# ru1ven/KeypointFusion

Hardware: AMD Instinct MI355X
Metric: RGB-D img/sec fwd (B=64, 256x256) (higher is better)
Workload: dtype f32; 1 GPU; KPFusion-convnext-tiny, depth+RGB UNet backbones forward, B=64/GPU 256x256 f32 (BASELINE configs[1]); batch_per_gpu=64, global_batch=64, input=256x256, parallelism=dp1 (batch shards, no collective)

## Files before the change

include/kpf.h:

```cpp
#ifndef KPF_H
#define KPF_H

#ifdef __cplusplus
extern "C" {
#endif

#define KPF_OK 0
#define KPF_EINVAL (-1)
#define KPF_ELAUNCH (-2)

#define KPF_DT_F32 0
#define KPF_DT_BF16 1
#define KPF_DT_F16 2
#define KPF_DT_F32_MMA_BF16 8
#define KPF_DT_F32_MMA_F16 9

#define KPF_ACT_RELU 1u
#define KPF_ACT_GELU 2u
#define KPF_RES_ADD 4u
#define KPF_RES_GAMMA 8u
#define KPF_RELU_AFTER_RES 16u
#define KPF_ACT_LEAKY 64u
#define KPF_IN_SPLIT 128u
#define KPF_W_SPLIT 512u
// ... 320 lines not shown
int kpf_geom_gate_uvd_forward(const float* pix_xyz, const float* joint_uvd, const float* par16, float* gam, int B, int J, int P, float half_size, float flip,
                              void* stream);
int kpf_geom_gate_uvd_backward(const float* pix_xyz, const float* joint_uvd, const float* par16, const float* dgam, float* djoint_uvd, int B, int J, int P,
                               float half_size, float flip, void* stream);

int kpf_prep_crop_u16(const unsigned char* rgb, const unsigned short* depth, const double* bbox, const double* cam, const double* cube, int B, int Hs, int Ws,
                      int x0, int y0, int H, int W, int S, float* img, float* img_rgb, float* center, float* M, float* cube_out, float* cam_para, double* com,
                      int* bounds, double* M64, void* stream);

int kpf_prep_pcl_sample(const float* img, const float* center, const double* M64, const double* cube, const double* cam, const long long* seed, int B, int S,
                        int n, float* pcl, int* pcl_index, int* pcl_count, float* cand_pts, void* stream);

int kpf_prep_uncrop_f32(const float* joints, const float* center, const float* M, const float* cube, const float* cam, int B, int J, float* crop_px,
                        float* frame_px, void* stream);

int kpf_prep_set_stamps(void* stamps64 );

int kpf_eval_errors_f32(const float* const* stages, int S, const float* gt, const float* cube, const int* score_index, int B, int J, int Jsel, float* err,
                        void* stream);

int kpf_eval_accumulate(const float* err, const unsigned char* valid, const double* thresholds, int S, int B, int Jsel, int T, long long* n_samples,
                        long long* n_batches, double* sum_err, double* sum_pa, double* sum_batch_mean, double* sum_batch_pa_mean, long long* pck,
                        long long* pck_pa, void* stream);

int kpf_prep_crop_u16_indexed(const unsigned char* rgb, const unsigned short* depth, const int* frame_index, int F, const double* bbox, const double* cam,
                              const double* cube, int B, int Hs, int Ws, int x0, int y0, int H, int W, int S, float* img, float* img_rgb, float* center, float* M,
                              float* cube_out, float* cam_para, double* com, int* bounds, double* M64, void* stream);

int kpf_track_step_f32(const float* joints, const float* center, const float* M, const float* cube, const float* cam_para, const int* pcl_count, int B, int J,
                       int frame_w, int frame_h, float expansion, long long seed_stride, double* bbox, long long* seed, int* lost, float* crop_px,
                       float* frame_px, float* cam_mm, double* bbox_used, int* status, void* stream);

int kpf_conv_num_tile_cfgs(void);

const char* kpf_last_error(void);
#define KPF_ABI_VERSION 21
int kpf_abi_version(void);

#ifdef __cplusplus
}
#endif
#endif
```

keypointfusion_amd/csrc/kpf_conv.hip:

```cpp
#include "kpf_common.h"
#include <stdlib.h>
#include <type_traits>

namespace {

struct ConvArgs {
  const float* in;
  const float* w;
  const float* bias;
  const float* ps;
  const float* pt;
  const float* gamma;
  const float* res;
  float* out;
  int M, N, K, Kp;
  int IH, IW, Cin, in_ld, in_coff;
  int OH, OW, ohow, KH, KW, sh, sw, ph, pw;
  int out_ld, out_coff, res_ld, res_coff;
  const float* zero;
  float w_unscale;
  unsigned flags;
  int tilesN, nblk;
  int vec;
  int dbg;
// ... 697 lines not shown
          blk[0] = h;
          blk[32] = (_Float16)(yc - (float)h);
        } else
          a.out[(long)m * a.out_ld + a.out_coff + n + e] = y;
      }
    }
  }
}

template <int TM, int TN, int WM, int WN, bool IS1X1, bool HAS_PRO, int EPI, int NS>
__global__ __launch_bounds__(64 * WM * WN) void igemm_f32_kernel(const ConvArgs a) {
  igemm_body<TM, TN, WM, WN, IS1X1, HAS_PRO, EPI, ARITH_F32, NS>(kpf_group_args(a));
}
template <int TM, int TN, int WM, int WN, bool IS1X1, int EPI, int ARITH>
__global__ __launch_bounds__(64 * WM * WN) void igemm_r16_kernel(const ConvArgs a) {
  igemm_body<TM, TN, WM, WN, IS1X1, false, EPI, ARITH, 2>(kpf_group_args(a));
}
template <int TM, int TN, int WM, int WN, bool IS1X1, bool HAS_PRO, int EPI, int ARITH, int NS>
__global__ __launch_bounds__(64 * WM * WN) void igemm_split_kernel(const ConvArgs a) {
  igemm_body<TM, TN, WM, WN, IS1X1, HAS_PRO, EPI, ARITH, NS>(kpf_group_args(a));
}
template <int TM, int TN, int WM, int WN, bool IS1X1, bool HAS_PRO, int EPI, int ARITH>
__global__ __launch_bounds__(64 * WM * WN, 4) void igemm_split_occ_kernel(const ConvArgs a) {
  igemm_body<TM, TN, WM, WN, IS1X1, HAS_PRO, EPI, ARITH, 1>(kpf_group_args(a));
}

template <int TM, int TN, int WM, int WN, bool IS1X1, bool HAS_PRO, int EPI, int ARITH, int NS>
__global__ __launch_bounds__(64 * WM * WN) void igemm_h16_kernel(const ConvArgs a) {
  igemm_body<TM, TN, WM, WN, IS1X1, HAS_PRO, EPI, ARITH, NS>(kpf_group_args(a));
}
template <int TM, int TN, int WM, int WN, bool IS1X1, bool HAS_PRO, int EPI, int ARITH>
__global__ __launch_bounds__(64 * WM * WN, 4) void igemm_h16_occ_kernel(const ConvArgs a) {
  igemm_body<TM, TN, WM, WN, IS1X1, HAS_PRO, EPI, ARITH, 1>(kpf_group_args(a));
}

template <int TM, int TN, int WM, int WN, bool IS1X1, bool HAS_PRO, int EPI, int ARITH, int NS>
int launch_one(const ConvArgs& a, hipStream_t st) {
  constexpr int BM = 16 * TM * WM, BN = 16 * TN * WN, RPP = 8 * WM * WN;
  constexpr bool R16 = ARITH == ARITH_R_BF16 || ARITH == ARITH_R_F16;
  constexpr bool WHOLE = NS > 2 || ARITH == ARITH_F32 || R16;
  constexpr int BMR = WHOLE ? (BM + RPP - 1) / RPP * RPP : BM, BNR = WHOLE ? (BN + RPP - 1) / RPP * RPP : BN;
  constexpr bool H16 = ARITH == ARITH_BF16 || ARITH == ARITH_F16;
  size_t lds = (size_t)(NS * (BMR + BNR) * BK + (HAS_PRO ? 2 * a.Kp * (H16 ? 2 : 1) : 0)) * sizeof(float);
  if (H16 && EPI != EPI_RES && EPI != EPI_GGRAD && TN == 4) {
    const size_t stg = (size_t)WM * WN * TM * 16 * (TN * 16 + 8) * 2;
    if (stg > lds) lds = stg;
  }
  void (*kern)(const ConvArgs);
  if constexpr (ARITH == ARITH_F32)
    kern = igemm_f32_kernel<TM, TN, WM, WN, IS1X1, HAS_PRO, EPI, NS>;
  else if constexpr (R16)
    kern = igemm_r16_kernel<TM, TN, WM, WN, IS1X1, EPI, ARITH>;
  else if constexpr (H16 && NS == 1)
    kern = igemm_h16_occ_kernel<TM, TN, WM, WN, IS1X1, HAS_PRO, EPI, ARITH>;
  else if constexpr (H16)
    kern = igemm_h16_kernel<TM, TN, WM, WN, IS1X1, HAS_PRO, EPI, ARITH, NS>;
  else if constexpr (NS == 1)
    kern = igemm_split_occ_kernel<TM, TN, WM, WN, IS1X1, HAS_PRO, EPI, ARITH>;
  else
    kern = igemm_split_kernel<TM, TN, WM, WN, IS1X1, HAS_PRO, EPI, ARITH, NS>;
  static std::atomic<bool> lds_opt_in[KPF_MAX_DEVICES];
  if (!kpf_raise_lds_limit(reinterpret_cast<const void*>(kern), lds_opt_in)) {
    kpf_set_error("kpf_conv2d_f32: cannot raise the dynamic LDS limit");
    return KPF_ELAUNCH;
  }
  if (lds > 160 * 1024) {
// ... 600 lines not shown
    }
  }
  static const bool no_kxk = getenv("KPF_NO_KXK16") != nullptr;
  if (!no_kxk && !pointwise && !pro_scale && a.groups <= 1 && !(fl & (KPF_RES_GELU_GRAD | KPF_ACT_GELU_SAVE | KPF_OUT_NCHW)) && a.M >= 16384) {
    const long tm256 = ((long)a.M + 255) / 256;
    if (a.N % 256 == 0 && tm256 * (a.N / 256) >= 256) best = 26;
    else if (a.N % 128 == 0 && tm256 * (a.N / 128) >= 256) best = 8;
    else if (a.N == 64) best = 2;
  }
  static const int forced = []() { const char* e = getenv("KPF_FORCE_CFG16"); return e ? atoi(e) : -1; }();
  if (forced >= 0 && (forced != 30 || ok8)) best = forced;
  if (d->tile_cfg > 0 && (d->tile_cfg != 31 || ok8)) best = d->tile_cfg - 1;
  if (best == 30) return dtype == KPF_DT_BF16 ? launch_8ph<ARITH_BF16>(a, st) : launch_8ph<ARITH_F16>(a, st);
#ifdef KPF_FAST_BUILD
  return launch_cfg_h16<4, 4, 2, 2, 2>(a, fast1x1, pointwise, dtype, st);
#endif
  switch (best) {
    case 0: return occ ? launch_cfg_h16<4, 4, 2, 2, 1>(a, fast1x1, pointwise, dtype, st) : launch_cfg_h16<4, 4, 2, 2, 2>(a, fast1x1, pointwise, dtype, st);
    case 1: return launch_cfg_h16<4, 3, 2, 2, 2>(a, fast1x1, pointwise, dtype, st);
    case 2: return launch_cfg_h16<2, 4, 4, 1, 2>(a, fast1x1, pointwise, dtype, st);
    case 5: return launch_cfg_h16<2, 4, 2, 2, 2>(a, fast1x1, pointwise, dtype, st);
    case 6: return occ ? launch_cfg_h16<2, 2, 2, 2, 1>(a, fast1x1, pointwise, dtype, st) : launch_cfg_h16<2, 2, 2, 2, 2>(a, fast1x1, pointwise, dtype, st);
    case 8: return launch_cfg_h16<4, 4, 4, 2, 2>(a, fast1x1, pointwise, dtype, st);
    case 20: return launch_cfg_h16<4, 4, 4, 2, 3>(a, fast1x1, pointwise, dtype, st);
    case 21: return launch_cfg_h16<4, 4, 2, 2, 3>(a, fast1x1, pointwise, dtype, st);
    case 22: return launch_cfg_h16<4, 4, 2, 2, 4>(a, fast1x1, pointwise, dtype, st);
    case 26: return launch_cfg_h16<8, 4, 2, 4, 2>(a, fast1x1, pointwise, dtype, st);
    case 41: return launch_cfg_h16<2, 2, 2, 2, 4>(a, fast1x1, pointwise, dtype, st);
    case 44: return launch_cfg_h16<2, 1, 1, 4, 8>(a, fast1x1, pointwise, dtype, st);
    default: return launch_cfg_h16<2, 1, 1, 4, 2>(a, fast1x1, pointwise, dtype, st);
  }
}
#else
extern "C" int kpf_conv2d_f32(const kpf_conv_desc* d, const float* in, const float* w, const float* bias,
                              const float* pro_scale, const float* pro_shift, const float* gamma, const float* res,
                              float* out, void* stream) {
  KPF_REQUIRE(d && in && w && out, "kpf_conv2d_f32: null pointer");
  KPF_REQUIRE(d->B > 0 && d->OH > 0 && d->OW > 0 && d->N > 0 && d->Cin > 0, "kpf_conv2d_f32: empty shape");
  KPF_REQUIRE(d->Cin % 4 == 0 && d->in_ld % 4 == 0 && d->in_coff % 4 == 0,
              "kpf_conv2d_f32: Cin/in_ld/in_coff must be multiples of 4 (got %d/%d/%d)", d->Cin, d->in_ld, d->in_coff);
  KPF_REQUIRE(d->Kp % 32 == 0 && d->Kp >= d->KH * d->KW * d->Cin, "kpf_conv2d_f32: Kp=%d must be a multiple of 32 and >= K=%d",
              d->Kp, d->KH * d->KW * d->Cin);
  KPF_REQUIRE(kpf_aligned16(in) && kpf_aligned16(w) && kpf_aligned16(out), "kpf_conv2d_f32: pointers must be 16-byte aligned");
  const unsigned fl = d->flags;
  if (!(fl & KPF_OUT_NCHW))
    KPF_REQUIRE(d->out_coff >= 0 && d->out_coff + d->N <= d->out_ld, "kpf_conv2d_f32: bad output slice ld=%d coff=%d N=%d",
                d->out_ld, d->out_coff, d->N);
  if (fl & KPF_RES_ADD)
    KPF_REQUIRE(res && kpf_aligned16(res) && d->res_coff >= 0 && d->res_coff + d->N <= d->res_ld, "kpf_conv2d_f32: bad residual");
  if (fl & KPF_RES_GAMMA) KPF_REQUIRE(gamma && (fl & KPF_RES_ADD), "kpf_conv2d_f32: RES_GAMMA needs gamma and RES_ADD");
  KPF_REQUIRE((pro_scale == nullptr) == (pro_shift == nullptr), "kpf_conv2d_f32: prologue needs both scale and shift");
  KPF_REQUIRE(((fl & KPF_ACT_RELU) != 0) + ((fl & KPF_ACT_GELU) != 0) + ((fl & KPF_ACT_LEAKY) != 0) <= 1, "kpf_conv2d_f32: one activation only");
  KPF_REQUIRE(!((fl & KPF_RES_ADD) && (fl & (KPF_ACT_RELU | KPF_ACT_GELU | KPF_ACT_LEAKY))), "kpf_conv2d_f32: activation before a residual add is not supported");
  KPF_REQUIRE(!((fl & KPF_ACT_LEAKY) && pro_scale), "kpf_conv2d_f32: LeakyReLU is not combined with an operand prologue");
  KPF_REQUIRE(!(fl & KPF_RELU_AFTER_RES) || (fl & KPF_RES_ADD), "kpf_conv2d_f32: RELU_AFTER_RES needs RES_ADD");
  KPF_REQUIRE(!(fl & KPF_RES_GELU_GRAD) || ((fl & KPF_RES_ADD) && !(fl & (KPF_RES_GAMMA | KPF_RELU_AFTER_RES | KPF_OUT_NCHW))), "kpf_conv2d_f32: RES_GELU_GRAD goes with RES_ADD alone");
  KPF_REQUIRE(!(fl & KPF_ACT_GELU_SAVE) || ((fl & KPF_ACT_GELU) && !(fl & (KPF_RES_ADD | KPF_OUT_NCHW)) && res && kpf_aligned16(res) && d->res_coff >= 0 && d->res_coff + d->N <= d->res_ld),
              "kpf_conv2d_f32: ACT_GELU_SAVE goes with ACT_GELU and a second output buffer in the res slot (res_ld / res_coff describe it)");
  KPF_REQUIRE((long)d->B * d->OH * d->OW < (1l << 31) && (long)d->B * d->IH * d->IW < (1l << 31), "kpf_conv2d_f32: too many pixels");

  ConvArgs a;
  a.in = in; a.w = w; a.bias = bias; a.ps = pro_scale; a.pt = pro_shift; a.gamma = gamma; a.res = res; a.out = out;
  a.M = d->B * d->OH * d->OW; a.N = d->N; a.K = d->KH * d->KW * d->Cin; a.Kp = d->Kp;
  a.IH = d->IH; a.IW = d->IW; a.Cin = d->Cin; a.in_ld = d->in_ld; a.in_coff = d->in_coff;
  a.OH = d->OH; a.OW = d->OW; a.ohow = d->OH * d->OW; a.KH = d->KH; a.KW = d->KW;
  a.sh = d->sh; a.sw = d->sw; a.ph = d->ph; a.pw = d->pw;
  a.out_ld = d->out_ld; a.out_coff = d->out_coff; a.res_ld = d->res_ld; a.res_coff = d->res_coff;
  {
    static const float* zero_of_dev[64] = {nullptr};
    int dev = 0;
    if (hipGetDevice(&dev) != hipSuccess || dev < 0 || dev >= 64) dev = 0;
    if (!zero_of_dev[dev]) {
      void* p = nullptr;
      if (hipGetSymbolAddress(&p, HIP_SYMBOL(kpf_zero16)) != hipSuccess || !p) {
        kpf_set_error("kpf_conv2d_f32: cannot resolve the zero page");
        return KPF_ELAUNCH;
      }
      zero_of_dev[dev] = static_cast<const float*>(p);
    }
    a.zero = zero_of_dev[dev];
  }
  a.flags = fl; a.tilesN = 0; a.nblk = 0; a.dbg = 0; a.skew = 0; a.st_policy = 0;
  {
    static const int st_mb = []() { const char* e = getenv("KPF_F32_ST_MB"); return e ? atoi(e) : 0; }();
    if (st_mb > 0 && (long)d->B * d->OH * d->OW * d->N * 4 >= (long)st_mb * 1000000) a.st_policy = 2;
  }
  a.w_unscale = (fl & (KPF_IN_SPLIT | KPF_W_SPLIT)) ? d->w_unscale : 1.0f;
  if (fl & (KPF_IN_SPLIT | KPF_W_SPLIT))
    KPF_REQUIRE(d->w_unscale > 0.f && d->Cin % 32 == 0 && d->in_coff % 4 == 0, "kpf_conv2d_f32: split operands need w_unscale > 0 and Cin %% 32 == 0 (Cin=%d)", d->Cin);
  if (fl & KPF_IN_SPLIT) KPF_REQUIRE(d->in_coff % 32 == 0 && d->in_ld % 32 == 0 && !pro_scale, "kpf_conv2d_f32: split activations need in_ld, in_coff multiples of 32 and no operand prologue");
  if (fl & KPF_OUT_SPLIT)
    KPF_REQUIRE(d->N % 32 == 0 && d->out_coff % 32 == 0 && d->out_ld % 32 == 0 && !(fl & KPF_OUT_NCHW),
                "kpf_conv2d_f32: split output needs N, out_ld, out_coff multiples of 32 (N=%d ld=%d coff=%d)", d->N, d->out_ld, d->out_coff);
  a.vec = (d->out_ld % 4 == 0 && d->out_coff % 4 == 0 && (!(fl & KPF_RES_ADD) || (d->res_ld % 4 == 0 && d->res_coff % 4 == 0))) ? 1 : 0;
  a.groups = d->groups > 1 ? d->groups : 1; a.g_in = a.g_out = 0; a.g_w = 0;
  if (a.groups > 1) {
    KPF_REQUIRE(!(fl & (KPF_RES_GAMMA | KPF_OUT_NCHW | KPF_IN_SPLIT | KPF_W_SPLIT | KPF_OUT_SPLIT)) && !pro_scale && d->w_gstride % 4 == 0,
                "kpf_conv2d_f32: a grouped launch takes no layer scale / prologue / NCHW output / split operands, and needs w_gstride %% 4 == 0");
    KPF_REQUIRE(d->in_coff + d->groups * d->Cin <= d->in_ld && d->out_coff + d->groups * d->N <= d->out_ld, "kpf_conv2d_f32: the groups' channel slices exceed the pixel stride");
    KPF_REQUIRE(!(fl & (KPF_RES_ADD | KPF_ACT_GELU_SAVE)) || d->res_coff + d->groups * d->N <= d->res_ld,
                "kpf_conv2d_f32: the groups' residual / saved pre-activation slices exceed the pixel stride");
    a.g_in = d->Cin; a.g_out = d->N; a.g_w = d->w_gstride;
    if ((d->out_coff + d->N) % 4 || ((fl & KPF_RES_ADD) && (d->res_coff + d->N) % 4)) a.vec = 0;
  }
  const bool is1x1 = d->KH == 1 && d->KW == 1 && d->sh == 1 && d->sw == 1 && d->ph == 0 && d->pw == 0 &&
                     d->IH == d->OH && d->IW == d->OW && d->Cin % 32 == 0 && d->Kp == d->Cin;
  hipStream_t st = reinterpret_cast<hipStream_t>(stream);

  int best = 0;
  double bc = 1e30;
  static const int forced = []() { const char* e = getenv("KPF_FORCE_CFG"); return e ? atoi(e) : -1; }();
  for (int i = 0; i < (int)(sizeof(kCfgs) / sizeof(kCfgs[0])); ++i) {
    const double c = cfg_cost(kCfgs[i], a.M, a.N, a.groups);
    if (c < bc) { bc = c; best = i; }
  }
  const bool f32_arith = !(fl & (KPF_IN_SPLIT | KPF_W_SPLIT));
  const bool gelu1x1 = f32_arith && is1x1 && (fl & KPF_ACT_GELU) && !(fl & KPF_ACT_GELU_SAVE) && !pro_scale && d->groups <= 1;
  if (gelu1x1 && a.M >= 1024 && a.N >= 512) {
    auto rounds_cost = [&](int bm, int bn, double pen) { return (double)((((long)(a.M + bm - 1) / bm) * ((a.N + bn - 1) / bn) + 255) / 256) * bm * bn * pen; };
    const double c0 = rounds_cost(128, 128, 1.00), c8 = rounds_cost(256, 128, 0.97);
    best = c0 <= c8 ? 0 : 8;
  }
  if (f32_arith && best < 9 && a.Kp >= 512) {
    const long bb = ((a.M + kCfgs[best].bm - 1) / kCfgs[best].bm) * ((a.N + kCfgs[best].bn - 1) / kCfgs[best].bn) * a.groups;
    if (bb < 256 && (long)((a.M + 31) / 32) * ((a.N + 63) / 64) * a.groups >= 512) best = 7;
  }
  if ((fl & (KPF_IN_SPLIT | KPF_W_SPLIT)) && !(fl & KPF_RES_ADD) && !pro_scale && (best == 0 || best == 8)) best = 13;
  if ((fl & (KPF_IN_SPLIT | KPF_W_SPLIT)) && !pro_scale && a.Kp >= 1024) {
    const long blocks = ((a.M + kCfgs[best < 9 ? best : 0].bm - 1) / kCfgs[best < 9 ? best : 0].bm) *
                        ((a.N + kCfgs[best < 9 ? best : 0].bn - 1) / kCfgs[best < 9 ? best : 0].bn);
    const long blocks64 = ((a.M + 63) / 64) * ((a.N + 63) / 64);
    if (best < 9 && blocks <= 512 && blocks64 >= 512) best = 16;
  }
  if (forced >= 0) best = forced;
  if (d->tile_cfg > 0) {
    KPF_REQUIRE(d->tile_cfg <= KPF_NUM_TILE_CFGS, "kpf_conv2d_f32: tile_cfg %d out of range", d->tile_cfg);
    best = d->tile_cfg - 1;
  }
#ifdef KPF_FAST_BUILD
  return launch_cfg<4, 4, 2, 2>(a, is1x1, st);
#else
  switch (best) {
    case 0: return launch_cfg<4, 4, 2, 2>(a, is1x1, st);
    case 1: return launch_cfg<4, 3, 2, 2>(a, is1x1, st);
    case 2: return launch_cfg<2, 4, 4, 1>(a, is1x1, st);
    case 3: return launch_cfg<4, 3, 4, 1>(a, is1x1, st);
    case 4: return launch_cfg<2, 7, 4, 1>(a, is1x1, st);
    case 5: return launch_cfg<2, 4, 2, 2>(a, is1x1, st);
    case 6: return launch_cfg<2, 2, 2, 2>(a, is1x1, st);
    case 8: return launch_cfg<4, 4, 4, 2>(a, is1x1, st);
    case 9: return launch_cfg<4, 4, 4, 2, 3>(a, is1x1, st);
    case 10: return launch_cfg<4, 4, 2, 2>(a, is1x1, st);
    case 11: return launch_cfg<4, 3, 2, 2>(a, is1x1, st);
    case 12: return launch_cfg<2, 4, 4, 1, 3>(a, is1x1, st);
    case 13: return launch_cfg<4, 4, 2, 2, 1>(a, is1x1, st);
    case 14: return launch_cfg<4, 3, 2, 2, 1>(a, is1x1, st);
    case 15: return launch_cfg<2, 4, 4, 1, 1>(a, is1x1, st);
    case 16: return launch_cfg<2, 2, 2, 2, 1>(a, is1x1, st);
    case 17: return launch_cfg<4, 6, 2, 2>(a, is1x1, st);
    default: return launch_cfg<2, 1, 1, 4>(a, is1x1, st);
  }
#endif
}

extern "C" int kpf_conv_num_tile_cfgs(void) { return KPF_NUM_TILE_CFGS; }
#endif

#ifdef KPF_DBG_TIME
extern "C" int kpf_dbg_read(unsigned long long* host, int n) {
  return hipMemcpyFromSymbol(host, HIP_SYMBOL(kpf_dbg_t), sizeof(unsigned long long) * n) == hipSuccess ? 0 : -1;
// ... 7 lines not shown
```

keypointfusion_amd/lib.py:

```python
import ctypes as C
import os

_HERE = os.path.dirname(os.path.abspath(__file__))
LIB_PATH = os.environ.get("KPF_LIB_PATH") or os.path.join(_HERE, "libkpf_hip.so")

KPF_ACT_RELU = 1
KPF_ACT_GELU = 2
KPF_RES_ADD = 4
KPF_RES_GAMMA = 8
KPF_RELU_AFTER_RES = 16
KPF_RES_GELU_GRAD = 1024
KPF_ACT_GELU_SAVE = 2048
KPF_PRO_LN = 4096
KPF_DT_F32_MMA_BF16, KPF_DT_F32_MMA_F16 = 8, 9
KPF_MMA_BF16, KPF_MMA_F16 = 8192, 16384
KPF_OUT_NCHW = 32
KPF_ACT_LEAKY = 64
KPF_IN_SPLIT = 128
KPF_OUT_SPLIT = 256
KPF_W_SPLIT = 512
KPF_DT_F32, KPF_DT_BF16, KPF_DT_F16 = 0, 1, 2
ABI_VERSION = 21


class ConvDesc(C.Structure):
    _fields_ = [(n, C.c_int) for n in (
        "B", "IH", "IW", "Cin", "in_ld", "in_coff", "OH", "OW", "N", "KH", "KW", "sh", "sw", "ph", "pw", "Kp",
        "out_ld", "out_coff", "res_ld", "res_coff")] + [("flags", C.c_uint), ("w_unscale", C.c_float), ("tile_cfg", C.c_int), ("groups", C.c_int), ("w_gstride", C.c_long)]


class PackDesc(C.Structure):
    _fields_ = [("src", C.c_void_p), ("dst", C.c_void_p)] + [(n, C.c_int) for n in (
        "N", "Cin", "KH", "KW", "mode", "n_pad", "Kp", "rows", "src_dtype", "dst_dtype", "first_block", "reserved")]


class AdamwDesc(C.Structure):
    _fields_ = [("p", C.c_void_p), ("g", C.c_void_p), ("m", C.c_void_p), ("v", C.c_void_p), ("n", C.c_long), ("first_block", C.c_int), ("reserved", C.c_int)]


class WgradGroupDesc(C.Structure):
    _fields_ = [("dy", C.c_void_p), ("x", C.c_void_p), ("dw", C.c_void_p), ("db", C.c_void_p), ("M", C.c_int), ("N", C.c_int), ("K", C.c_int), ("first_block", C.c_int), ("sps", C.c_int), ("ldy", C.c_int)]


class ColsumDesc(C.Structure):
    _fields_ = [("part", C.c_void_p), ("dw", C.c_void_p), ("db", C.c_void_p), ("nblk", C.c_int), ("C", C.c_int), ("first_block", C.c_int), ("reserved", C.c_int)]


class WgradReduceDesc(C.Structure):
    _fields_ = [("part", C.c_void_p), ("dbpart", C.c_void_p), ("dw", C.c_void_p), ("db", C.c_void_p), ("g_ws", C.c_long)] + [
        (n, C.c_int) for n in "S N K Cin KHW nkb ndb groups Cin_out N_out kind first_block".split()]


_P = C.c_void_p
_SIGS = {
    "kpf_conv2d_f32": [C.POINTER(ConvDesc), _P, _P, _P, _P, _P, _P, _P, _P, _P],
# ... 18 lines not shown
    "kpf_slices_sum_relu_backward": [_P, _P, _P, _P, C.c_long, C.c_int, C.c_int, C.c_int, _P],
    "kpf_group_max_train_forward": [_P, _P, _P, C.c_long, C.c_int, C.c_int, _P],
    "kpf_group_max_train_backward": [_P, C.c_int, _P, _P, C.c_long, C.c_int, C.c_int, _P],
    "kpf_heat_gam_gate_f32": [_P, _P, _P, C.c_int] + [_P] * 10 + [C.c_int] * 4 + [_P],
    "kpf_gate_reduce_f32": [_P, _P, _P, _P, _P, C.c_int, C.c_int, _P],
    "kpf_tr_encoder_f32": [_P, C.c_int, C.c_int, _P, _P, _P, _P, C.c_int, C.c_int, _P],
    "kpf_xattn_layer_f32": [_P, _P, _P, _P, C.c_int, C.c_int, C.c_int, _P],
    "kpf_conv2d_h16": [C.POINTER(ConvDesc), _P, _P, _P, _P, _P, _P, _P, _P, C.c_int, _P],
    "kpf_conv2d_h16_uses_8ph": [C.POINTER(ConvDesc), C.c_int],
    "kpf_conv2d_h16_ln_fold_supported": [C.POINTER(ConvDesc)],
    "kpf_dwconv7_ln_h16": [_P, _P, _P, _P, _P, _P, C.c_int, C.c_int, C.c_int, C.c_int, C.c_float, C.c_int, _P],
    "kpf_layernorm_h16": [_P, C.c_int, _P, _P, _P, C.c_int, C.c_long, C.c_int, C.c_float, _P],
    "kpf_upsample2x_h16": [_P, _P, C.c_int, C.c_int, C.c_int, C.c_int, C.c_int, C.c_int, C.c_int, _P],
    "kpf_cast_h16_f32": [_P, C.c_int, _P, C.c_long, C.c_int, C.c_int, C.c_int, _P],
    "kpf_cast_f32_h16": [_P, _P, C.c_int, C.c_long, _P],
    "kpf_convnext_mlp_f32": [_P] * 8 + [C.c_long, C.c_int, _P],
    "kpf_convnext_mlp_supported": [C.c_int],
    "kpf_convnext_mlp_split_f32": [_P, _P, _P, _P, C.c_float, _P, _P, C.c_float, _P, _P, C.c_long, C.c_int, _P],
    "kpf_convnext_mlp_split_supported": [C.c_int],
    "kpf_convnext_mlp_h16": [_P] * 8 + [C.c_long, C.c_int, C.c_int, _P],
    "kpf_convnext_mlp_h16_supported": [C.c_int],
    "kpf_dwconv7_stats_h16": [_P, _P, _P, _P, _P, C.c_int, C.c_int, C.c_int, C.c_int, C.c_int, _P],
    "kpf_dwconv7_stats_supported": [C.c_int, C.c_int, C.c_int],
    "kpf_ln_apply_stats_h16": [_P, _P, _P, _P, C.c_long, C.c_int, C.c_float, C.c_int, _P],
    "kpf_ln_stats_merge": [_P, _P, C.c_long, C.c_int, C.c_float, _P],
    "kpf_cbam_channel_gate_f32": [_P] * 7 + [C.c_int] * 4 + [_P],
    "kpf_cbam_spatial_gate_f32": [_P, _P, _P, C.c_float, C.c_float, _P, _P, C.c_int, C.c_int, C.c_int, C.c_int, _P],
    "kpf_cbam_apply_f32": [_P] * 5 + [C.c_int] * 3 + [_P],
    "kpf_maxpool2x2_f32": [_P, _P, C.c_int, C.c_int, C.c_int, C.c_int, _P],
    "kpf_upnearest2x_add_f32": [_P, _P, _P, C.c_int, C.c_int, C.c_int, C.c_int, _P],
    "kpf_mano_forward_f32": [_P, C.c_int, _P, C.c_int] + [_P] * 10 + [C.c_int, _P],
    "kpf_tr_encoder_weight_floats": [C.c_int],
    "kpf_conv_num_tile_cfgs": [],
    "kpf_xattn_weight_floats": [],
    "kpf_bn_train_forward": [_P, C.c_int, _P, _P, _P, C.c_int, _P, _P, _P, _P, C.c_float, C.c_float, C.c_int, _P, C.c_long, C.c_long, C.c_int, _P],
    "kpf_bn_train_backward": [_P, _P, _P, C.c_int, C.c_int, _P, _P, _P, _P, _P, _P, _P, C.c_int, _P, C.c_long, C.c_long, C.c_int, _P],
    "kpf_dwconv7_f32": [_P, _P, _P, _P, C.c_int, C.c_int, C.c_int, C.c_int, _P],
    "kpf_dwconv7_add_f32": [_P, _P, _P, _P, _P, C.c_int, C.c_int, C.c_int, C.c_int, _P],
    "kpf_conv2d_wgrad": [_P, _P, C.c_int] + [_P] * 3 + [C.c_long] + [C.c_int] * 18 + [C.POINTER(WgradReduceDesc), _P],
    "kpf_dwconv7_wgrad": [_P] * 5 + [C.c_long] + [C.c_int] * 4 + [C.POINTER(WgradReduceDesc), _P],
    "kpf_wgrad_reduce_multi": [C.POINTER(WgradReduceDesc), C.c_int, _P],
    "kpf_row_gather_cols_f32": [_P, C.c_long, C.c_long, C.c_long, _P, _P, _P, C.c_int, C.c_int, C.c_int, C.c_int, C.c_int, _P],
    "kpf_bn_ssr_forward": [_P] * 7 + [C.c_float, C.c_float, _P, C.c_long, C.c_long, C.c_int, C.c_int, C.c_int, _P],
    "kpf_bn_ssr_backward": [_P] * 10 + [C.c_long, C.c_long, C.c_int, C.c_int, C.c_int, _P],
    "kpf_bn_relu_gmax_forward": [_P] * 8 + [C.c_float, C.c_float, _P, C.c_long, C.c_long, C.c_int, C.c_int, _P],
    "kpf_bn_relu_gmax_backward": [_P, C.c_int] + [_P] * 9 + [C.c_long, C.c_long, C.c_int, C.c_int, _P],
    "kpf_bn2_add_relu_forward": [_P] * 12 + [C.c_float, C.c_float, _P, C.c_long, C.c_long, C.c_int, _P],
    "kpf_bn2_add_relu_backward": [_P] * 14 + [C.c_long, C.c_long, C.c_int, _P],
    "kpf_unstack_rows": [_P, C.c_int, _P, C.c_long, C.c_int, C.c_int, C.c_int, C.c_int, C.c_int, _P],
    "kpf_restack_rows": [C.POINTER(C.c_void_p), _P, C.c_int, C.c_long, C.c_int, C.c_int, C.c_int, C.c_int, C.c_int, _P],
    "kpf_add_relu_forward": [_P, _P, _P, _P, C.c_long, C.c_float, _P],
    "kpf_add_relu_backward": [_P, _P, _P, C.c_long, C.c_float, _P],
    "kpf_gate_mix_forward": [_P] * 6 + [C.c_int] * 3 + [_P],
    "kpf_gate_mix_backward": [_P] * 11 + [C.c_int] * 3 + [_P],
    "kpf_pad_rows": [_P, C.c_int, _P, C.c_int, C.c_long, C.c_int, C.c_int, C.c_int, _P],
    "kpf_pose_tokens_f32": [_P, _P, _P, _P, C.c_int, C.c_int, C.c_int, C.c_int, C.c_float, _P],
    "kpf_upsample2x_bwd": [_P, _P] + [C.c_int] * 5 + [_P],
    "kpf_maxpool3x3s2_fwd": [_P, _P, _P] + [C.c_int] * 5 + [_P],
    "kpf_maxpool3x3s2_bwd": [_P, _P, _P] + [C.c_int] * 5 + [_P],
    "kpf_row_gather_fwd_f32": [_P] * 4 + [C.c_int] * 5 + [_P],
    "kpf_pack_conv_weight": [_P, C.c_int, _P, C.c_int] + [C.c_int] * 7 + [_P],
    "kpf_pack_conv_weights_multi": [_P, C.c_int, C.c_int, _P],
    "kpf_joint_heatmap_forward": [_P, _P, C.c_int, C.c_int, C.c_int, C.c_float, C.c_float, _P],
    "kpf_joint_heatmap_backward": [_P, _P, _P, C.c_int, C.c_int, C.c_int, C.c_float, C.c_float, _P],
    "kpf_geom_gate_forward": [_P, _P, _P, C.c_int, C.c_int, C.c_int, _P],
    "kpf_geom_gate_backward": [_P, _P, _P, _P, C.c_int, C.c_int, C.c_int, _P],
# ... 107 lines not shown
```

Before: 3538 img/s.

## Add persistent f32 1x1 GELU igemm kernel overlapping epilogue with next tile

```diff
diff --git a/include/kpf.h b/include/kpf.h
--- a/include/kpf.h
+++ b/include/kpf.h
@@ -376,9 +376,10 @@
                        float* frame_px, float* cam_mm, double* bbox_used, int* status, void* stream);
 
 int kpf_conv_num_tile_cfgs(void);
+int kpf_conv2d_f32_is_persistent(const kpf_conv_desc* d, int has_prologue);
 
 const char* kpf_last_error(void);
-#define KPF_ABI_VERSION 21
+#define KPF_ABI_VERSION 22
 int kpf_abi_version(void);
 
 #ifdef __cplusplus
diff --git a/keypointfusion_amd/csrc/kpf_conv.hip b/keypointfusion_amd/csrc/kpf_conv.hip
--- a/keypointfusion_amd/csrc/kpf_conv.hip
+++ b/keypointfusion_amd/csrc/kpf_conv.hip
@@ -753,6 +753,242 @@
 template <int TM, int TN, int WM, int WN, bool IS1X1, bool HAS_PRO, int EPI, int ARITH>
 __global__ __launch_bounds__(64 * WM * WN, 4) void igemm_h16_occ_kernel(const ConvArgs a) {
   igemm_body<TM, TN, WM, WN, IS1X1, HAS_PRO, EPI, ARITH, 1>(kpf_group_args(a));
+}
+
+template <int TM, int TN, int WM, int WN, bool NT>
+__global__ __launch_bounds__(64 * WM * WN) void igemm_f32_persistent_kernel(const ConvArgs a) {
+  constexpr int BM = 16 * TM * WM, BN = 16 * TN * WN, NW = WM * WN, RPP = 8 * NW, AP = BM / RPP, BP = BN / RPP, TILE = (BM + BN) * BK;
+  static_assert(BM % RPP == 0 && BN % RPP == 0, "whole staging passes");
+  static_assert((TM * (112 / TM)) == 112, "the epilogue slice is spread over the 112 MFMAs in front of the barrier");
+  extern __shared__ __attribute__((aligned(16))) float lds[];
+
+  const int tid = threadIdx.x;
+  const int lane = tid & 63;
+  const int wave = __builtin_amdgcn_readfirstlane(tid >> 6);
+  const int wm = wave % WM, wn = wave / WM;
+  KPF_STAMP(0);
+  const int G = gridDim.x, X = G < 8 ? G : 8;
+  const int xcd = blockIdx.x % X;
+  const int W = (G - xcd + X - 1) / X;
+  int tile, tend;
+  {
+    const int q = a.nblk / X, r = a.nblk % X;
+    const int first = xcd < r ? xcd * (q + 1) : r * (q + 1) + (xcd - r) * q;
+    tile = first + (int)blockIdx.x / X;
+    tend = first + q + (xcd < r ? 1 : 0);
+  }
+  if (tile >= tend) return;
+
+  const int nk = a.Kp / BK;
+  const int fr = lane & 15, fg = lane >> 4, rsw = (fr >> 1) & 7;
+  const int lr = tid >> 3;
+  const int kc = (((tid & 7) ^ ((lr >> 1) & 7)) << 2);
+  const float* const in_lane = a.in + (long)lr * a.in_ld + a.in_coff + kc;
+  const float* const w_lane = a.w + (long)lr * a.Kp + kc;
+  float* const out_lane = a.out + (long)(wm * TM * 16 + fr) * a.out_ld + a.out_coff + wn * TN * 16 + fg * 4;
+  const float* const bias_lane = a.bias ? a.bias + wn * TN * 16 + fg * 4 : a.zero;
+  const int bstep = a.bias ? 1 : 0;
+  const long a_pass = (long)RPP * a.in_ld, b_pass = (long)RPP * a.Kp;
+
+  auto stage = [&](int buf, const float* sa, const float* sb) {
+    float* As = lds + buf * TILE;
+    float* Bs = As + BM * BK;
+#pragma unroll
+    for (int p = 0; p < AP; ++p)
+      __builtin_amdgcn_global_load_lds((gbl_void_t*)(sa + p * a_pass), (lds_void_t*)(As + (RPP * p + 8 * wave) * BK), 16, 0, 0);
+#pragma unroll
+    for (int p = 0; p < BP; ++p)
+      __builtin_amdgcn_global_load_lds((gbl_void_t*)(sb + p * b_pass), (lds_void_t*)(Bs + (RPP * p + 8 * wave) * BK), 16, 0, 0);
+  };
+  auto read_frags = [&](int buf, int s16, f32x4(&xf)[TM], f32x4(&wf)[TN]) {
+    const float* xrow = lds + buf * TILE + (wm * TM * 16 + fr) * BK;
+    const float* wrow = lds + buf * TILE + BM * BK + (wn * TN * 16 + fr) * BK;
+    const int sc = (((4 * s16 + fg) ^ rsw) << 2);
+#pragma unroll
+    for (int j = 0; j < TM; ++j) xf[j] = *reinterpret_cast<const f32x4*>(xrow + j * 16 * BK + sc);
+#pragma unroll
+    for (int i = 0; i < TN; ++i) wf[i] = *reinterpret_cast<const f32x4*>(wrow + i * 16 * BK + sc);
+  };
+  auto mma = [&](int e, const f32x4(&xf)[TM], const f32x4(&wf)[TN], f32x4(&acc)[TN][TM]) {
+#pragma unroll
+    for (int i = 0; i < TN; ++i)
+#pragma unroll
+      for (int j = 0; j < TM; ++j) acc[i][j] = __builtin_amdgcn_mfma_f32_16x16x4f32(wf[i][e], xf[j][e], acc[i][j], 0, 0, 0);
+  };
+  auto store4 = [&](float* p, const f32x4& v) {
+    if constexpr (NT) __builtin_nontemporal_store(v, reinterpret_cast<f32x4*>(p));
+    else STORE4(p, v);
+  };
+
+  int stile = tile, sg = 0;
+  const float *sa, *sb;
+  auto seek = [&](int t) {
+    const int nt = t % a.tilesN, mt = t / a.tilesN;
+    sa = in_lane + (long)(mt * BM) * a.in_ld;
+    sb = w_lane + (long)(nt * BN) * a.Kp;
+  };
+  auto advance = [&]() {
+    if (++sg == nk) {
+      sg = 0;
+      if (stile + W < tend) stile += W;
+      seek(stile);
+    } else {
+      sa += BK;
+      sb += BK;
+    }
+  };
+
+  int m0 = 0, n0 = 0;
+  float* out_prev = nullptr;
+  const float* bias_prev = bias_lane;
+  const float* bias_cur = bias_lane;
+  f32x4 bq = {0.f, 0.f, 0.f, 0.f};
+  f32x4 xa[TM], wa[TN], xb[TM], wb[TN];
+  int buf = 0;
+
+  auto kiter = [&](auto slice_c, auto bias_c, f32x4(&ac)[TN][TM], const f32x4(&ap)[TN][TM]) {
+    constexpr int S = decltype(slice_c)::value, BIAS = decltype(bias_c)::value;
+    read_frags(buf, 1, xb, wb);
+    f32x4 bqn;
+    {
+      const float* bp = BIAS == 1 ? bias_prev + bstep * (S + 1) * 16 : bias_cur;
+      asm volatile("global_load_dwordx4 %0, %1, off" : "=&v"(bqn) : "v"(bp) : "memory");
+    }
+    if constexpr (S >= 0) {
+#pragma unroll
+      for (int j = 0; j < TM; ++j) {
+        f32x4 v = ap[S][j];
+#pragma unroll
+        for (int e = 0; e < 4; ++e) {
+          float y = gelu_erf(v[e] + bq[e]);
+          asm("" : "+v"(y));
+          v[e] = y;
+        }
+        store4(out_prev + (long)(j * 16) * a.out_ld + S * 16, v);
+      }
+    }
+#pragma unroll
+    for (int e = 0; e < 4; ++e) mma(e, xa, wa, ac);
+#pragma unroll
+    for (int e = 0; e < 3; ++e) mma(e, xb, wb, ac);
+    if constexpr (S >= 0) {
+      __builtin_amdgcn_sched_group_barrier(0x100, TM + TN, 0);
+#pragma unroll
+      for (int j = 0; j < TM; ++j) {
+#pragma unroll
+        for (int g = 0; g < 112 / TM; ++g) {
+          __builtin_amdgcn_sched_group_barrier(0x008, 1, 0);
+          __builtin_amdgcn_sched_group_barrier(0x402, 3, 0);
+        }
+        __builtin_amdgcn_sched_group_barrier(0x040, 1, 0);
+      }
+    }
+    __builtin_amdgcn_sched_barrier(0);
+    asm volatile("s_waitcnt vmcnt(0) lgkmcnt(0)" : "+v"(bqn) : : "memory");
+    __builtin_amdgcn_s_barrier();
+    __builtin_amdgcn_sched_barrier(0);
+    bq = bqn;
+    read_frags(buf ^ 1, 0, xa, wa);
+    stage(buf, sa, sb);
+    mma(3, xb, wb, ac);
+    __builtin_amdgcn_sched_group_barrier(0x100, TM + TN, 0);
+#pragma unroll
+    for (int q = 0; q < AP + BP; ++q) {
+      __builtin_amdgcn_sched_group_barrier(0x008, (TM * TN) / (AP + BP) > 0 ? (TM * TN) / (AP + BP) : 1, 0);
+      __builtin_amdgcn_sched_group_barrier(0x020, 1, 0);
+    }
+    advance();
+    buf ^= 1;
+  };
+  auto run_tile = [&](auto defer_c, f32x4(&ac)[TN][TM], const f32x4(&ap)[TN][TM]) {
+    constexpr bool DEFER = decltype(defer_c)::value;
+    const f32x4 zero4 = {0.f, 0.f, 0.f, 0.f};
+#pragma unroll
+    for (int i = 0; i < TN; ++i)
+#pragma unroll
+      for (int j = 0; j < TM; ++j) ac[i][j] = zero4;
+    using std::integral_constant;
+    int kt = 0;
+    if constexpr (DEFER) {
+      static_assert(TN == 4, "one peeled K iteration per channel quad");
+      kiter(integral_constant<int, 0>(), integral_constant<int, 1>(), ac, ap);
+      kiter(integral_constant<int, 1>(), integral_constant<int, 1>(), ac, ap);
+      kiter(integral_constant<int, 2>(), integral_constant<int, 1>(), ac, ap);
+      kiter(integral_constant<int, 3>(), integral_constant<int, 2>(), ac, ap);
+      kt = TN;
+    }
+    for (; kt < nk; ++kt) kiter(integral_constant<int, -1>(), integral_constant<int, 2>(), ac, ap);
+  };
+  auto plain_epilogue = [&](const f32x4(&acc)[TN][TM]) {
+    f32x4 bvv[TN];
+#pragma unroll
+    for (int i = 0; i < TN; ++i) bvv[i] = *reinterpret_cast<const f32x4*>(bias_cur + bstep * i * 16);
+    float* o = out_lane + (long)m0 * a.out_ld + n0;
+#pragma unroll
+    for (int j = 0; j < TM; ++j)
+#pragma unroll
+      for (int i = 0; i < TN; ++i) {
+        f32x4 v = acc[i][j];
+#pragma unroll
+        for (int e = 0; e < 4; ++e) v[e] = gelu_erf(v[e] + bvv[i][e]);
+        store4(o + (long)(j * 16) * a.out_ld + i * 16, v);
+      }
+  };
+  auto enter = [&](int t) {
+    out_prev = out_lane + (long)m0 * a.out_ld + n0;
+    bias_prev = bias_cur;
+    n0 = (t % a.tilesN) * BN;
+    m0 = (t / a.tilesN) * BM;
+    bias_cur = bias_lane + bstep * n0;
+  };
+
+  f32x4 accA[TN][TM], accB[TN][TM];
+  enter(tile);
+  seek(tile);
+  stage(0, sa, sb);
+  advance();
+  __syncthreads();
+  KPF_STAMP(1);
+  read_frags(0, 0, xa, wa);
+  stage(1, sa, sb);
+  advance();
+  run_tile(std::false_type(), accA, accB);
+  for (;;) {
+    tile += W;
+    if (tile >= tend) {
+      KPF_STAMP(2);
+      plain_epilogue(accA);
+      break;
+    }
+    enter(tile);
+    run_tile(std::true_type(), accB, accA);
+    tile += W;
+    if (tile >= tend) {
+      KPF_STAMP(2);
+      plain_epilogue(accB);
+      break;
+    }
+    enter(tile);
+    run_tile(std::true_type(), accA, accB);
+  }
+  asm volatile("s_waitcnt vmcnt(0)" ::: "memory");
+  KPF_STAMP(3);
+}
+
+template <int TM, int TN, int WM, int WN>
+int launch_persistent(ConvArgs& a, int grid, hipStream_t st) {
+  constexpr int BM = 16 * TM * WM, BN = 16 * TN * WN;
+  a.tilesN = a.N / BN;
+  a.nblk = (a.M / BM) * a.tilesN;
+  const size_t lds = (size_t)2 * (BM + BN) * BK * sizeof(float);
+  void (*kern)(const ConvArgs) = a.st_policy == 2 ? igemm_f32_persistent_kernel<TM, TN, WM, WN, true> : igemm_f32_persistent_kernel<TM, TN, WM, WN, false>;
+  static std::atomic<bool> lds_opt_in[2][KPF_MAX_DEVICES];
+  if (!kpf_raise_lds_limit(reinterpret_cast<const void*>(kern), lds_opt_in[a.st_policy == 2 ? 1 : 0])) {
+    kpf_set_error("kpf_conv2d_f32: cannot raise the dynamic LDS limit");
+    return KPF_ELAUNCH;
+  }
+  hipLaunchKernelGGL(kern, dim3(grid), dim3(64 * WM * WN), lds, st, a);
+  return kpf_check_launch("kpf_conv2d_f32");
 }
 
 template <int TM, int TN, int WM, int WN, bool IS1X1, bool HAS_PRO, int EPI, int ARITH, int NS>
@@ -1419,6 +1655,83 @@
   }
 }
 #else
+static int pick_cfg_f32(const kpf_conv_desc* d, long M, int groups, bool has_pro, bool is1x1) {
+  const long N = d->N;
+  const int Kp = d->Kp;
+  int best = 0;
+  double bc = 1e30;
+  static const int forced = []() { const char* e = getenv("KPF_FORCE_CFG"); return e ? atoi(e) : -1; }();
+  for (int i = 0; i < (int)(sizeof(kCfgs) / sizeof(kCfgs[0])); ++i) {
+    const double c = cfg_cost(kCfgs[i], M, N, groups);
+    if (c < bc) { bc = c; best = i; }
+  }
+  const unsigned fl = d->flags;
+  const bool f32_arith = !(fl & (KPF_IN_SPLIT | KPF_W_SPLIT));
+  const bool gelu1x1 = f32_arith && is1x1 && (fl & KPF_ACT_GELU) && !(fl & KPF_ACT_GELU_SAVE) && !has_pro && d->groups <= 1;
+  if (gelu1x1 && M >= 1024 && N >= 512) {
+    auto rounds_cost = [&](int bm, int bn, double pen) { return (double)((((long)(M + bm - 1) / bm) * ((N + bn - 1) / bn) + 255) / 256) * bm * bn * pen; };
+    const double c0 = rounds_cost(128, 128, 1.00), c8 = rounds_cost(256, 128, 0.97);
+    best = c0 <= c8 ? 0 : 8;
+  }
+  if (f32_arith && best < 9 && Kp >= 512) {
+    const long bb = ((M + kCfgs[best].bm - 1) / kCfgs[best].bm) * ((N + kCfgs[best].bn - 1) / kCfgs[best].bn) * groups;
+    if (bb < 256 && (long)((M + 31) / 32) * ((N + 63) / 64) * groups >= 512) best = 7;
+  }
+  if ((fl & (KPF_IN_SPLIT | KPF_W_SPLIT)) && !(fl & KPF_RES_ADD) && !has_pro && (best == 0 || best == 8)) best = 13;
+  if ((fl & (KPF_IN_SPLIT | KPF_W_SPLIT)) && !has_pro && Kp >= 1024) {
+    const long blocks = ((M + kCfgs[best < 9 ? best : 0].bm - 1) / kCfgs[best < 9 ? best : 0].bm) *
+                        ((N + kCfgs[best < 9 ? best : 0].bn - 1) / kCfgs[best < 9 ? best : 0].bn);
+    const long blocks64 = ((M + 63) / 64) * ((N + 63) / 64);
+    if (best < 9 && blocks <= 512 && blocks64 >= 512) best = 16;
+  }
+  if (forced >= 0) best = forced;
+  if (d->tile_cfg > 0) best = d->tile_cfg - 1;
+  return best;
+}
+
+static int kpf_cu_count() {
+  static std::atomic<int> cus[KPF_MAX_DEVICES];
+  int dev = 0, n = 0;
+  if (hipGetDevice(&dev) != hipSuccess || dev < 0 || dev >= KPF_MAX_DEVICES) return 256;
+  if ((n = cus[dev].load(std::memory_order_relaxed)) > 0) return n;
+  if (hipDeviceGetAttribute(&n, hipDeviceAttributeMultiprocessorCount, dev) != hipSuccess || n <= 0) return 256;
+  cus[dev].store(n, std::memory_order_relaxed);
+  return n;
+}
+
+static int persistent_grid_f32(const kpf_conv_desc* d, long M, bool has_pro, bool is1x1, int vec, int best) {
+  if (best != 8) return 0;
+  const char* v1 = getenv("KPF_IGEMM_V1");
+  if (v1 && atoi(v1) != 0) return 0;
+  const unsigned fl = d->flags;
+  if (fl & (KPF_IN_SPLIT | KPF_W_SPLIT | KPF_OUT_SPLIT | KPF_OUT_NCHW | KPF_ACT_GELU_SAVE)) return 0;
+  if (!(fl & KPF_ACT_GELU) || !is1x1 || has_pro || d->groups > 1 || !vec) return 0;
+  if (M % 256 != 0 || d->N % 128 != 0 || d->Kp < 128) return 0;
+  const long tiles = (M / 256) * (d->N / 128);
+  int grid = kpf_cu_count();
+  const char* pg = getenv("KPF_IGEMM_PGRID");
+  if (pg && atoi(pg) > 0 && atoi(pg) < grid) grid = atoi(pg);
+  return tiles > grid ? grid : 0;
+}
+
+static bool dense_1x1_f32(const kpf_conv_desc* d) {
+  return d->KH == 1 && d->KW == 1 && d->sh == 1 && d->sw == 1 && d->ph == 0 && d->pw == 0 && d->IH == d->OH && d->IW == d->OW && d->Cin % 32 == 0 && d->Kp == d->Cin;
+}
+static int vec_rows_f32(const kpf_conv_desc* d) {
+  const unsigned fl = d->flags;
+  int vec = (d->out_ld % 4 == 0 && d->out_coff % 4 == 0 && (!(fl & KPF_RES_ADD) || (d->res_ld % 4 == 0 && d->res_coff % 4 == 0))) ? 1 : 0;
+  if (d->groups > 1 && ((d->out_coff + d->N) % 4 || ((fl & KPF_RES_ADD) && (d->res_coff + d->N) % 4))) vec = 0;
+  return vec;
+}
+
+extern "C" int kpf_conv2d_f32_is_persistent(const kpf_conv_desc* d, int has_prologue) {
+  if (!d || d->B <= 0 || d->OH <= 0 || d->OW <= 0 || d->N <= 0 || d->Kp <= 0 || d->Kp % 32 != 0 || d->tile_cfg > KPF_NUM_TILE_CFGS) return 0;
+  const long M = (long)d->B * d->OH * d->OW;
+  const bool is1x1 = dense_1x1_f32(d);
+  const int best = pick_cfg_f32(d, M, d->groups > 1 ? d->groups : 1, has_prologue != 0, is1x1);
+  return persistent_grid_f32(d, M, has_prologue != 0, is1x1, vec_rows_f32(d), best) > 0 ? 1 : 0;
+}
+
 extern "C" int kpf_conv2d_f32(const kpf_conv_desc* d, const float* in, const float* w, const float* bias,
                               const float* pro_scale, const float* pro_shift, const float* gamma, const float* res,
                               float* out, void* stream) {
@@ -1469,7 +1782,8 @@
   }
   a.flags = fl; a.tilesN = 0; a.nblk = 0; a.dbg = 0; a.skew = 0; a.st_policy = 0;
   {
-    static const int st_mb = []() { const char* e = getenv("KPF_F32_ST_MB"); return e ? atoi(e) : 0; }();
+    const char* e = getenv("KPF_F32_ST_MB");
+    const int st_mb = e ? atoi(e) : 0;
     if (st_mb > 0 && (long)d->B * d->OH * d->OW * d->N * 4 >= (long)st_mb * 1000000) a.st_policy = 2;
   }
   a.w_unscale = (fl & (KPF_IN_SPLIT | KPF_W_SPLIT)) ? d->w_unscale : 1.0f;
@@ -1479,7 +1793,7 @@
   if (fl & KPF_OUT_SPLIT)
     KPF_REQUIRE(d->N % 32 == 0 && d->out_coff % 32 == 0 && d->out_ld % 32 == 0 && !(fl & KPF_OUT_NCHW),
                 "kpf_conv2d_f32: split output needs N, out_ld, out_coff multiples of 32 (N=%d ld=%d coff=%d)", d->N, d->out_ld, d->out_coff);
-  a.vec = (d->out_ld % 4 == 0 && d->out_coff % 4 == 0 && (!(fl & KPF_RES_ADD) || (d->res_ld % 4 == 0 && d->res_coff % 4 == 0))) ? 1 : 0;
+  a.vec = vec_rows_f32(d);
   a.groups = d->groups > 1 ? d->groups : 1; a.g_in = a.g_out = 0; a.g_w = 0;
   if (a.groups > 1) {
     KPF_REQUIRE(!(fl & (KPF_RES_GAMMA | KPF_OUT_NCHW | KPF_IN_SPLIT | KPF_W_SPLIT | KPF_OUT_SPLIT)) && !pro_scale && d->w_gstride % 4 == 0,
@@ -1488,41 +1802,17 @@
     KPF_REQUIRE(!(fl & (KPF_RES_ADD | KPF_ACT_GELU_SAVE)) || d->res_coff + d->groups * d->N <= d->res_ld,
                 "kpf_conv2d_f32: the groups' residual / saved pre-activation slices exceed the pixel stride");
     a.g_in = d->Cin; a.g_out = d->N; a.g_w = d->w_gstride;
-    if ((d->out_coff + d->N) % 4 || ((fl & KPF_RES_ADD) && (d->res_coff + d->N) % 4)) a.vec = 0;
-  }
-  const bool is1x1 = d->KH == 1 && d->KW == 1 && d->sh == 1 && d->sw == 1 && d->ph == 0 && d->pw == 0 &&
-                     d->IH == d->OH && d->IW == d->OW && d->Cin % 32 == 0 && d->Kp == d->Cin;
+  }
+  const bool is1x1 = dense_1x1_f32(d);
   hipStream_t st = reinterpret_cast<hipStream_t>(stream);
 
-  int best = 0;
-  double bc = 1e30;
-  static const int forced = []() { const char* e = getenv("KPF_FORCE_CFG"); return e ? atoi(e) : -1; }();
-  for (int i = 0; i < (int)(sizeof(kCfgs) / sizeof(kCfgs[0])); ++i) {
-    const double c = cfg_cost(kCfgs[i], a.M, a.N, a.groups);
-    if (c < bc) { bc = c; best = i; }
-  }
-  const bool f32_arith = !(fl & (KPF_IN_SPLIT | KPF_W_SPLIT));
-  const bool gelu1x1 = f32_arith && is1x1 && (fl & KPF_ACT_GELU) && !(fl & KPF_ACT_GELU_SAVE) && !pro_scale && d->groups <= 1;
-  if (gelu1x1 && a.M >= 1024 && a.N >= 512) {
-    auto rounds_cost = [&](int bm, int bn, double pen) { return (double)((((long)(a.M + bm - 1) / bm) * ((a.N + bn - 1) / bn) + 255) / 256) * bm * bn * pen; };
-    const double c0 = rounds_cost(128, 128, 1.00), c8 = rounds_cost(256, 128, 0.97);
-    best = c0 <= c8 ? 0 : 8;
-  }
-  if (f32_arith && best < 9 && a.Kp >= 512) {
-    const long bb = ((a.M + kCfgs[best].bm - 1) / kCfgs[best].bm) * ((a.N + kCfgs[best].bn - 1) / kCfgs[best].bn) * a.groups;
-    if (bb < 256 && (long)((a.M + 31) / 32) * ((a.N + 63) / 64) * a.groups >= 512) best = 7;
-  }
-  if ((fl & (KPF_IN_SPLIT | KPF_W_SPLIT)) && !(fl & KPF_RES_ADD) && !pro_scale && (best == 0 || best == 8)) best = 13;
-  if ((fl & (KPF_IN_SPLIT | KPF_W_SPLIT)) && !pro_scale && a.Kp >= 1024) {
-    const long blocks = ((a.M + kCfgs[best < 9 ? best : 0].bm - 1) / kCfgs[best < 9 ? best : 0].bm) *
-                        ((a.N + kCfgs[best < 9 ? best : 0].bn - 1) / kCfgs[best < 9 ? best : 0].bn);
-    const long blocks64 = ((a.M + 63) / 64) * ((a.N + 63) / 64);
-    if (best < 9 && blocks <= 512 && blocks64 >= 512) best = 16;
-  }
-  if (forced >= 0) best = forced;
-  if (d->tile_cfg > 0) {
-    KPF_REQUIRE(d->tile_cfg <= KPF_NUM_TILE_CFGS, "kpf_conv2d_f32: tile_cfg %d out of range", d->tile_cfg);
-    best = d->tile_cfg - 1;
+  if (d->tile_cfg > 0) KPF_REQUIRE(d->tile_cfg <= KPF_NUM_TILE_CFGS, "kpf_conv2d_f32: tile_cfg %d out of range", d->tile_cfg);
+  const int best = pick_cfg_f32(d, a.M, a.groups, pro_scale != nullptr, is1x1);
+  {
+    const int pgrid = persistent_grid_f32(d, a.M, pro_scale != nullptr, is1x1, a.vec, best);
+    const float *ib = in + d->in_coff, *ie = in + (long)(a.M - 1) * d->in_ld + d->in_coff + d->Cin;
+    const float *ob = out + d->out_coff, *oe = out + (long)(a.M - 1) * d->out_ld + d->out_coff + d->N;
+    if (pgrid > 0 && !(ib < oe && ob < ie)) return launch_persistent<4, 4, 4, 2>(a, pgrid, st);
   }
 #ifdef KPF_FAST_BUILD
   return launch_cfg<4, 4, 2, 2>(a, is1x1, st);
diff --git a/keypointfusion_amd/lib.py b/keypointfusion_amd/lib.py
--- a/keypointfusion_amd/lib.py
+++ b/keypointfusion_amd/lib.py
@@ -20,7 +20,7 @@
 KPF_OUT_SPLIT = 256
 KPF_W_SPLIT = 512
 KPF_DT_F32, KPF_DT_BF16, KPF_DT_F16 = 0, 1, 2
-ABI_VERSION = 21
+ABI_VERSION = 22
 
 
 class ConvDesc(C.Structure):
@@ -105,6 +105,7 @@
     "kpf_mano_forward_f32": [_P, C.c_int, _P, C.c_int] + [_P] * 10 + [C.c_int, _P],
     "kpf_tr_encoder_weight_floats": [C.c_int],
     "kpf_conv_num_tile_cfgs": [],
+    "kpf_conv2d_f32_is_persistent": [C.POINTER(ConvDesc), C.c_int],
     "kpf_xattn_weight_floats": [],
     "kpf_bn_train_forward": [_P, C.c_int, _P, _P, _P, C.c_int, _P, _P, _P, _P, C.c_float, C.c_float, C.c_int, _P, C.c_long, C.c_long, C.c_int, _P],
     "kpf_bn_train_backward": [_P, _P, _P, C.c_int, C.c_int, _P, _P, _P, _P, _P, _P, _P, C.c_int, _P, C.c_long, C.c_long, C.c_int, _P],
```

Result: no change. 3554 img/s, median of 6 (+0.4%).
